# lubaroli/sigsvgd

Hardware: AMD Instinct MI355X
Metric: SVGD iters/sec, sig-kernel N=1024 T=64 d=7 (higher is better)
Workload: dtype f64 static kernel + f32 sweeps and contraction (mixed), f32 I/O

## Files before the change

### sigsvgd_amd/csrc/gram_fast.hip

```cpp
#include <cstdlib>

#include "gram_fast_kernel.h"

namespace sigsvgd {

bool fast_supported(int T, int d, int n) { return n == 0 && T >= 3 && T <= 64 && d <= 16; }
bool fast_wide_supported(int T, int d, int n) { return n == 0 && T >= 3 && T <= 64 && d >= 17 && d <= 32; }

namespace {
inline int grad_nw(int T, int d) { return (d <= 8) ? 8 : 4; }
inline int grad_wg_per_cu(int T, int d) { return (d <= 8 && T <= 32) ? 3 : 1; }
GradGeom fast_geometry(int A, int B, int T, int d, bool sym, int off, int stride, bool fold)
{
    return grad_geometry(A, B, T * d, sym, off, stride, fold, grad_nw(T, d), (long long)device_cu_count() * grad_wg_per_cu(T, d));
}
}

int sym_tile_rows_fast(int T, int d) { return grad_nw(T, d); }

static bool fixed_windows(int T, int want_grad)
{
    if (T != 64 || !want_grad) return false;
    const char *e = getenv("SIGSVGD_SWEEP_WINDOWS");
    return !(e && e[0] == 't');
}

static bool wave_balance(int T, int d, int want_grad, bool sym)
{
    if (!sym || d > 8 || !fast_has_balance<8, true>() || !fixed_windows(T, want_grad)) return false;
    const char *e = getenv("SIGSVGD_WAVE_BALANCE");
    return !(e && e[0] == 'o' && e[1] == 'f');
}

static bool half_offset(int T, int d, int want_grad, bool sym)
{
    if (!sym || d != 7 || !fast_has_half<8, true, true>() || !fixed_windows(T, want_grad)) return false;
    const char *e = getenv("SIGSVGD_HALF_OFFSET");
    return !(e && e[0] == 'o' && e[1] == 'f');
}

WsPlan fast_plan(int A, int B, int T, int d, int want_grad, bool sym, int off, int stride, bool fold, int kind)
{
    WsPlan w;
    const bool rbf = kind == SIGSVGD_STATIC_RBF;
    w.fixed_windows = rbf && d <= 16 && fixed_windows(T, want_grad) ? 1 : 0;
    w.wave_balance = rbf && wave_balance(T, d, want_grad, sym) ? 1 : 0;
    w.half_offset = rbf && half_offset(T, d, want_grad, sym) ? 1 : 0;
    if (d <= 4) w.kflag = w.take(flag_area_bytes(A, B));
    if (want_grad) {
        w.g = fast_geometry(A, B, T, d, sym, off, stride, fold);
        w.rseg = w.take(w.g.rseg_bytes);
        w.cslab = w.take(w.g.cslab_bytes);
    }
    return w;
}

namespace {
int run(const GramProblem &p, const WsPlan &w, bool sym, const TileMap &own, void *out, int out64)
{
    unsigned char *base = nullptr;
    int rc = ws_base(p, w, "fast", base);
    if (rc) return rc;
    FastArgs a{};
    fill_sweep_args(a, p, w, base);
    a.tm = own;
    int tile_rows = 0;
    rc = p.kind != SIGSVGD_STATIC_RBF ? fast_radial_dispatch(p, a, w, out != nullptr, sym, tile_rows)
         : p.d > 16                   ? fast_wide_dispatch(p, a, w, out != nullptr, sym, tile_rows)
                                      : dispatch_variant<0>(p, a, w, out != nullptr, sym, tile_rows);
    if (rc) return rc;
    return finish_launch(p, w, base, sym, a.tm, tile_rows, out, out64);
}
}

int fast_launch(const GramProblem &p)
{
    const bool sym = (p.flags & SIGSVGD_FLAG_Y_IS_X) && p.A == p.B;
    const WsPlan w = fast_plan(p.A, p.B, p.T, p.d, p.gradX_out != nullptr, sym, 0, 1, false, p.kind);
    return run(p, w, sym, make_tilemap(1, 0, 1, false), p.gradX_out, p.dtype == SIGSVGD_F64);
}

int fast_sym_partial(const GramProblem &p, int tile_offset, int tile_stride, bool fold, double *grad_partial)
{
    const WsPlan w = fast_plan(p.A, p.B, p.T, p.d, 1, true, tile_offset, tile_stride, fold, p.kind);
    return run(p, w, true, make_tilemap((p.A + grad_nw(p.T, p.d) - 1) / grad_nw(p.T, p.d), tile_offset, tile_stride, fold),
               grad_partial, 1);
}

}

SIG_EXEC_DEBUG_GETTER(fast)
```

### sigsvgd_amd/csrc/gram_fast_kernel.h

```cpp
#pragma once

#include <type_traits>

#include "sig_common.h"

namespace sigsvgd {

#define SIG_PRIO(n)                                                          \
    if (!GRAD || !SYM || (RING == 32 && NW == 4)) __builtin_amdgcn_s_setprio(n);

template <int BAL>
__device__ __forceinline__ void bal_top(bool first)
{
    if constexpr (BAL != 0) {
        if (first) __builtin_amdgcn_s_setprio(1);
    }
}
template <int BAL, int AT>
__device__ __forceinline__ void bal_switch(bool first)
{
    if constexpr (BAL != 0 && (BAL & 3) == AT) {
        if (first) __builtin_amdgcn_s_setprio(0);
        else __builtin_amdgcn_s_setprio(1);
    }
// ... 253 lines not shown
                     : [cur] "+v"(cur), [upA] "+v"(upA), [upB] "+v"(upB), [V] "+v"(V), [t] "=&v"(t), [y] "=&v"(y),
                       [k0] "+v"(ksl[0]), [k1] "+v"(ksl[1]), [k2] "+v"(ksl[2]), [k3] "+v"(ksl[3]), [k4] "+v"(ksl[4]),
                       [k5] "+v"(ksl[5]), [k6] "+v"(ksl[6]), [k7] "+v"(ksl[7])
                     : [g0] "v"(g[0]), [g1] "v"(g[1]), [g2] "v"(g[2]), [g3] "v"(g[3]), [g4] "v"(g[4]), [g5] "v"(g[5]),
                       [g6] "v"(g[6]), [g7] "v"(g[7]), [r3] "s"(r3), SIG_WIN_OPS(0), SIG_WIN_OPS(1), SIG_WIN_OPS(2),
                       SIG_WIN_OPS(3), SIG_WIN_OPS(4), SIG_WIN_OPS(5), SIG_WIN_OPS(6), SIG_WIN_OPS(7));
    else
        asm volatile(SIG_FWD_STEP_X("upA", "upB", "g0", SIG_FWD_KSL("upB", "k0"), SIG_WIN_FIX("0"))
                     SIG_FWD_STEP_X("upB", "upA", "g1", SIG_FWD_KSL("upA", "k1"), SIG_WIN_FIX("1"))
                     SIG_FWD_STEP_X("upA", "upB", "g2", SIG_FWD_KSL("upB", "k2"), SIG_WIN_FIX("2"))
                     SIG_FWD_STEP_X("upB", "upA", "g3", SIG_FWD_KSL("upA", "k3"), SIG_WIN_FIX("3"))
                     SIG_FWD_STEP_X("upA", "upB", "g4", SIG_FWD_KSL("upB", "k4"), SIG_WIN_FIX("4"))
                     "s_mov_b64 exec, -1\n\t"
                     : [cur] "+v"(cur), [upA] "+v"(upA), [upB] "+v"(upB), [V] "+v"(V), [t] "=&v"(t), [y] "=&v"(y),
                       [k0] "+v"(ksl[0]), [k1] "+v"(ksl[1]), [k2] "+v"(ksl[2]), [k3] "+v"(ksl[3]), [k4] "+v"(ksl[4])
                     : [g0] "v"(g[0]), [g1] "v"(g[1]), [g2] "v"(g[2]), [g3] "v"(g[3]), [g4] "v"(g[4]), [r3] "s"(r3),
                       SIG_WIN_OPS(0), SIG_WIN_OPS(1), SIG_WIN_OPS(2), SIG_WIN_OPS(3), SIG_WIN_OPS(4));
}
template <int PFIX, int SIGMA0, int NS>
__device__ __forceinline__ void sweep_rev_fixed(float &cur, float &dnA, float &dnB, float &V, const float *g, float *ksl, const float r3)
{
    static_assert((NS == 8 || NS == 5) && SIGMA0 % 8 == 0 && SIGMA0 + NS <= 2 * PFIX - 1, "statement shape");
    float t, y;
    SIG_EXEC_MUST_BE_FULL("sweep_rev_fixed");
    if constexpr (NS == 8)
        asm volatile(SIG_REV_STEP_X("dnA", "dnB", "g7", "k7", SIG_WIN_FIX("7")) SIG_REV_STEP_X("dnB", "dnA", "g6", "k6", SIG_WIN_FIX("6"))
                     SIG_REV_STEP_X("dnA", "dnB", "g5", "k5", SIG_WIN_FIX("5")) SIG_REV_STEP_X("dnB", "dnA", "g4", "k4", SIG_WIN_FIX("4"))
                     SIG_REV_STEP_X("dnA", "dnB", "g3", "k3", SIG_WIN_FIX("3")) SIG_REV_STEP_X("dnB", "dnA", "g2", "k2", SIG_WIN_FIX("2"))
                     SIG_REV_STEP_X("dnA", "dnB", "g1", "k1", SIG_WIN_FIX("1")) SIG_REV_STEP_X("dnB", "dnA", "g0", "k0", SIG_WIN_FIX("0"))
                     "s_mov_b64 exec, -1\n\t"
                     : [cur] "+v"(cur), [dnA] "+v"(dnA), [dnB] "+v"(dnB), [V] "+v"(V), [t] "=&v"(t), [y] "=&v"(y),
                       [k0] "+v"(ksl[0]), [k1] "+v"(ksl[1]), [k2] "+v"(ksl[2]), [k3] "+v"(ksl[3]), [k4] "+v"(ksl[4]),
                       [k5] "+v"(ksl[5]), [k6] "+v"(ksl[6]), [k7] "+v"(ksl[7])
                     : [g0] "v"(g[0]), [g1] "v"(g[1]), [g2] "v"(g[2]), [g3] "v"(g[3]), [g4] "v"(g[4]), [g5] "v"(g[5]),
                       [g6] "v"(g[6]), [g7] "v"(g[7]), [r3] "s"(r3), SIG_WIN_OPS(0), SIG_WIN_OPS(1), SIG_WIN_OPS(2),
                       SIG_WIN_OPS(3), SIG_WIN_OPS(4), SIG_WIN_OPS(5), SIG_WIN_OPS(6), SIG_WIN_OPS(7));
    else
        asm volatile(SIG_REV_STEP_X("dnB", "dnA", "g4", "k4", SIG_WIN_FIX("4"))
                     SIG_REV_STEP_X("dnA", "dnB", "g3", "k3", SIG_WIN_FIX("3")) SIG_REV_STEP_X("dnB", "dnA", "g2", "k2", SIG_WIN_FIX("2"))
                     SIG_REV_STEP_X("dnA", "dnB", "g1", "k1", SIG_WIN_FIX("1")) SIG_REV_STEP_X("dnB", "dnA", "g0", "k0", SIG_WIN_FIX("0"))
                     "s_mov_b64 exec, -1\n\t"
                     : [cur] "+v"(cur), [dnA] "+v"(dnA), [dnB] "+v"(dnB), [V] "+v"(V), [t] "=&v"(t), [y] "=&v"(y),
                       [k0] "+v"(ksl[0]), [k1] "+v"(ksl[1]), [k2] "+v"(ksl[2]), [k3] "+v"(ksl[3]), [k4] "+v"(ksl[4])
                     : [g0] "v"(g[0]), [g1] "v"(g[1]), [g2] "v"(g[2]), [g3] "v"(g[3]), [g4] "v"(g[4]), [r3] "s"(r3),
                       SIG_WIN_OPS(0), SIG_WIN_OPS(1), SIG_WIN_OPS(2), SIG_WIN_OPS(3), SIG_WIN_OPS(4));
}
template <int PFIX, int S0, int S1>
__device__ __forceinline__ void sweep_fwd_fixed_round(float &cur, float &upA, float &upB, float &V, const float *Dsl, float *Ksl, const float r3)
{
    if constexpr (S0 < S1) {
        sweep_fwd_fixed<PFIX, S0, (S1 - S0 < 8 ? S1 - S0 : 8)>(cur, upA, upB, V, Dsl + (S0 & 63), Ksl + (S0 & 63), r3);
        sweep_fwd_fixed_round<PFIX, S0 + 8, S1>(cur, upA, upB, V, Dsl, Ksl, r3);
    }
}
template <int PFIX, int S0, int S1>
__device__ __forceinline__ void sweep_rev_fixed_round(float &cur, float &dnA, float &dnB, float &V, const float *Dsl, float *Ksl, const float r3)
{
    if constexpr (S0 < S1) {
        sweep_rev_fixed_round<PFIX, S0 + 8, S1>(cur, dnA, dnB, V, Dsl, Ksl, r3);
        sweep_rev_fixed<PFIX, S0, (S1 - S0 < 8 ? S1 - S0 : 8)>(cur, dnA, dnB, V, Dsl + (S0 & 63), Ksl + (S0 & 63), r3);
    }
}

template <int RING>
__device__ __forceinline__ double resweep_fwd_fp64(const float (&Dsl)[RING], int P, int lrow)
{
    double cur = 1.0, upprev = 1.0;
    asm volatile("" : "+v"(lrow), "+s"(P));
    const bool rowv = lrow < P;
#pragma unroll
    for (int s0 = 0; s0 < 2 * RING - 3; s0 += 8) {
        if (s0 <= 2 * P - 2) {
#pragma unroll
            for (int s = s0; s < s0 + 8 && s < 2 * RING - 3; ++s) {
                const double up = dpp_shr1_one(cur);
                float gf = Dsl[s & (RING - 1)];
                asm volatile("" : "+v"(gf));
                const double g = (double)gf;
                const double t = cur + up;
                const double nw = (t - upprev) + g * __builtin_fma(g, t + upprev, 1.7320508075688772 * t);
                cur = (rowv && (unsigned)(s - lrow) < (unsigned)P) ? nw : cur;
                upprev = up;
            }
        }
    }
    return cur;
}

__device__ __forceinline__ double rsqrt_ge1(double x)
{
    const double y = __builtin_amdgcn_rsq(x);
    const double e = __builtin_fma(-(x * y), y, 1.0);
    return __builtin_fma(y * e, __builtin_fma(e, 0.375, 0.5), y);
}

constexpr int GS_STRIDE = 65;
constexpr int GS_WAVE = 64 * GS_STRIDE;
using f32x2 = __attribute__((ext_vector_type(2))) float;

__device__ __forceinline__ int gs_index(int slot, int lane) { return slot * GS_STRIDE + lane; }

template <int DPAD, int NW, bool GRAD, bool SYM, bool LP, int RING = 64, int PFIX = 0, int BAL = 0, int RADIAL = 0, int HALF = 0>
__global__ __launch_bounds__(NW * 64) __attribute__((amdgpu_waves_per_eu(
    GRAD ? ((RING == 32 && NW == 4 && DPAD <= 8) ? 3 : 1) : ((DPAD <= 8) ? 3 : (DPAD <= 16) ? 2 : 1),
    GRAD ? ((RING == 32 && NW == 4 && DPAD <= 8) ? 3 : (DPAD <= 16) ? 2 : 1) : ((DPAD <= 8) ? 3 : (DPAD <= 16) ? 2 : 1)))) void gram_fast_kernel(FastArgsOf<RADIAL> a)
{
    constexpr int DC = LP ? DPAD - 1 : DPAD;
    constexpr int NT = NW * 64;
    constexpr int RM = RING - 1;
    constexpr int RPW = (RING == 32) ? 2 : 1;
    constexpr int NWR = NW * RPW;
    static_assert(RADIAL == 0 || (PFIX == 0 && BAL == 0), "the radial kinds: general windows, no wave balance");
    static_assert(BAL == 0 || (GRAD && SYM && RING == 64 && NW == 8 && PFIX != 0 && (BAL & 3) != 0 && BAL < 8),
                  "wave balance: the symmetric gradient kernels with fixed windows on 8-wave workgroups (the ones SIG_PRIO leaves alone)");
    static_assert(HALF == 0 || (GRAD && SYM && LP && DPAD == 8 && RING == 64 && NW == 8 && PFIX != 0 && BAL == 0 && RADIAL == 0),
                  "half offset: the symmetric 7-of-8-channel gradient kernel with fixed windows on 8-wave workgroups; a schedule of its own");
    constexpr int YDS = DPAD + 2;
    constexpr int YFS = (DPAD == 4) ? 12 : DPAD + 4;
    constexpr int GSS = HALF ? 64 : GS_STRIDE;
    constexpr int GSW = RING * GSS;
    __shared__ float Gs_all[GRAD ? NW * GSW : 1];
    __shared__ __align__(16) double yd[2 * RING * YDS];
    __shared__ double ynd[HALF ? 1 : 2 * RING];
    constexpr int YFB = 2 * RING * YFS;
    __shared__ double yref[HALF ? 2 * DPAD : DPAD];
    __shared__ __align__(16) float yf[GRAD ? (HALF ? 2 : 1) * YFB : 1];
    __shared__ float ypark[HALF ? (NW / 2) * RING * DC : 1];
    __shared__ float ycarry[HALF ? RING * DC : 1];

    const int tid = threadIdx.x, lane = tid & 63;
    const int wave = __builtin_amdgcn_readfirstlane(tid >> 6);
    const int lrow = lane & RM;
    const bool bal_first = (BAL & 4) ? wave < NW / 2 : wave >= NW / 2;
    const bool half_younger = HALF != 0 && wave >= NW / 2;
    int pb = 0;
    const int T = a.T, d = a.d, P = T - 1, io64 = a.io64;
#ifdef SIGSVGD_PHASE_STAMPS
    unsigned long long ph_[SIG_FAST_PHASES] = {0, 0, 0, 0, 0, 0, 0, 0, 0}, tlast_ = __builtin_amdgcn_s_memtime();
#endif
    int j0 = 0, j1 = 0;
    float *Gs = Gs_all + (GRAD ? wave * GSW : 0);
    const double inv_h = a.inv_h;
    const float m2h = (float)(-2.0 * inv_h * 3.46410161513775459);

    float Ksl[RING];
    double gacc[DPAD];
    double xraw[DPAD];

    constexpr int EPT = (64 * DPAD + NT - 1) / NT;
    constexpr bool RAW_STAGE = GRAD && SYM && RING == 64 && DPAD == 8;
    struct RawElem { unsigned lo, hi; };
    RawElem raw_v[EPT], raw_r[EPT];
    double stage_v[EPT], stage_r[EPT];
    auto load_raw = [&](const void *b, size_t idx) -> RawElem {
        const char *p = static_cast<const char *>(b) + (idx << (io64 ? 3 : 2));
        RawElem r;
        r.lo = *reinterpret_cast<const unsigned *>(p);
        r.hi = 0u;
        if (io64) r.hi = *reinterpret_cast<const unsigned *>(p + 4);
        return r;
    };
    auto raw_value = [&](const RawElem &r) -> double {
        return io64 ? __hiloint2double((int)r.hi, (int)r.lo) : (double)__uint_as_float(r.lo);
    };
    auto stage_load = [&](int j) {
#pragma unroll
        for (int k = 0; k < EPT; ++k) {
            const int e = tid + k * NT;
            const int t = e / DPAD, c = e % DPAD;
            const bool ok = e < RING * DPAD && t < T && c < d && j < a.B;
            if constexpr (RAW_STAGE) {
                raw_v[k] = raw_r[k] = RawElem{0u, 0u};
                if (ok) {
                    raw_v[k] = load_raw(a.Y, ((size_t)j * T + t) * d + c);
                    raw_r[k] = load_raw(a.Y, (size_t)j * T * d + c);
                }
            } else {
                stage_v[k] = ok ? load_any(a.Y, ((size_t)j * T + t) * d + c, io64) : 0.0;
                stage_r[k] = ok ? load_any(a.Y, (size_t)j * T * d + c, io64) : 0.0;
            }
        }
    };
    const double nscale = RADIAL ? inv_h : -inv_h * 1.4426950408889634074;
    auto stage_store = [&](int buf) {
#pragma unroll
        for (int k = 0; k < EPT; ++k) {
            const int e = tid + k * NT;
            if (e < RING * DPAD) {
                const int t = e / DPAD, c = e % DPAD;
                if constexpr (RAW_STAGE) {
                    stage_v[k] = raw_value(raw_v[k]);
                    stage_r[k] = raw_value(raw_r[k]);
                }
                const double v = stage_v[k] - stage_r[k];
                if (!(LP && c == DPAD - 1)) {
                    yd[t * YDS + c] = v;
                    yd[(t + RING) * YDS + c] = v;
                }
                if (GRAD) {
                    float *yfb = yf + (HALF ? buf * YFB : 0);
                    yfb[t * YFS + c] = (float)v;
                    yfb[(t + RING) * YFS + c] = (float)v;
                }
                if (t == 0) yref[(HALF ? buf * DPAD : 0) + c] = stage_r[k];
                double s = v * v * nscale;
#pragma unroll
                for (int off = 1; off < DPAD; off <<= 1) s += __shfl_xor(s, off, 64);
                if (c == 0) {
                    if constexpr (!HALF) {
                        ynd[t] = s;
                        ynd[t + RING] = s;
                    }
                    if (LP) {
                        yd[t * YDS + DPAD - 1] = s;
                        yd[(t + RING) * YDS + DPAD - 1] = s;
                    }
                }
            }
        }
    };

    const long long it0 = a.nitems * blockIdx.x / gridDim.x, it1 = a.nitems * (blockIdx.x + 1) / gridDim.x;
    int remaining = (int)(it1 - it0);
    long long item = it0;
    int kq = 0, cstart = 0;
    {
        long long rem = it0;
        for (;; ++kq) {
            const int cn = a.B - (SYM ? a.tm.tile_of(kq) * NWR : 0);
            if (rem < cn) break;
            rem -= cn;
        }
        cstart = (int)rem;
    }
    bool staged = false;
    while (remaining > 0) {
    const int itile = a.tm.tile_of(kq);
    const int cfirst = SYM ? itile * NWR : 0;
    const int ncol = min(a.B - cfirst - cstart, remaining);
    const int jnext_tile = SYM ? a.tm.tile_of(kq + 1) * NWR : 0;
    const bool more_tiles = remaining > ncol;
    const int i0 = itile * NWR + wave * RPW;
    const int i = (RING == 32) ? i0 + (lane >> 5) : i0;
    const bool row_ok = i < a.A;
#pragma unroll
    for (int c = 0; c < DPAD; ++c) {
        gacc[c] = 0.0;
        xraw[c] = (row_ok && lrow < T && c < d) ? load_any(a.X, ((size_t)i * T + lrow) * d + c, io64) : 0.0;
    }
    if constexpr (RAW_STAGE) {
#pragma unroll
        for (int c = 0; c < DPAD; ++c) asm volatile("" : "+v"(xraw[c]));
    }
    j0 = cfirst + cstart;
    j1 = j0 + ncol;
    if (!staged) {
        staged = true;
        stage_load(j0);
        stage_store(pb);
        __syncthreads();
    }

    for (int j = j0; j < j1; ++j) {
        const bool pair_ok = i0 < a.A && (!SYM || j >= i0);
        const bool mine = row_ok && (!SYM || j >= i);
        const bool last = j + 1 == j1;
        const bool more = !last || more_tiles;
        if (more) stage_load(last ? jnext_tile : j + 1);

        float Dsl[RING];
        const double *yrefp = yref + (HALF ? pb * DPAD : 0);
        auto pair_sync = [&]() __attribute__((always_inline)) {
            SIG_STAMP(5)
#ifndef SIG_EXPERIMENT_NO_PAIR_BARRIER
            __syncthreads();
#endif
            SIG_STAMP(6)
            if constexpr (HALF != 0) {
                const float inv_d = 1.0f / (float)d;
                const bool pend = j > j0;
                float *dstp = a.cslab + (size_t)(item - 1) * (T * d);
                for (int e = tid; e < T * d; e += NT) {
                    const int n = (int)(((float)e + 0.5f) * inv_d), c = e - n * d;
                    if (pend) {
                        float s = ycarry[e];
#pragma unroll
                        for (int w = 0; w < NW / 2; ++w) s += ypark[w * RING * DC + e];
                        dstp[e] = s;
                    }
                    float s = 0.f;
#pragma unroll
                    for (int w = 0; w < NW / 2; ++w) s += Gs_all[w * GSW + n * DPAD + c];
                    ycarry[e] = s;
                }
            } else if (GRAD && SYM) {
                const float inv_d = 1.0f / (float)d;
                float *dst = a.cslab + (size_t)item * (T * d);
                for (int e = tid; e < T * d; e += NT) {
                    const int n = (int)(((float)e + 0.5f) * inv_d), c = e - n * d;
                    float s = 0.f;
#pragma unroll
                    for (int w = 0; w < NW; ++w) {
                        s += Gs_all[w * GSW + n * DPAD + c];
                        if (RING == 32) s += Gs_all[w * GSW + (RING + n) * DPAD + c];
                    }
                    dst[e] = s;
                }
            }
            ++item;
            if (more) stage_store(HALF ? pb ^ 1 : 0);
            SIG_STAMP(7)
#ifndef SIG_EXPERIMENT_NO_PAIR_BARRIER
            __syncthreads();
#endif
            SIG_STAMP(8)
        };
        auto younger_sync = [&]() __attribute__((always_inline)) {
            if constexpr (RAW_STAGE) {
#pragma unroll
                for (int k = 0; k < EPT; ++k)
                    asm volatile("" : "+v"(raw_v[k].lo), "+v"(raw_v[k].hi), "+v"(raw_r[k].lo), "+v"(raw_r[k].hi));
            }
            pair_sync();
        };

        SIG_STAMP(0)
        SIG_PRIO(3)
        if (pair_ok) {
            bal_top<BAL>(bal_first);
            double xs[DPAD];
            double xn = 0.0;
#pragma unroll
            for (int c = 0; c < DPAD; ++c) {
                const double xc = (lrow < T && c < d) ? xraw[c] - yrefp[c] : 0.0;
                xn = __builtin_fma(xc, xc, xn);
                xs[c] = xc * (-2.0 * nscale);
            }
// ... 243 lines not shown
                    const unsigned long long *mk = (RING == 64 ? SWEEP_MASK.m[P] : SWEEP_MASK32.m[P]) + rnd * 64;
#pragma unroll
                    for (int k0 = 56; k0 >= 0; k0 -= 8) sweep_rev8(cur, downA, downB, V, &Dsl[k0 & RM], &Ksl[k0 & RM], mk + k0, r3);
                }

                if constexpr (DPAD == 4) {
                    if (a.kflag) {
                        float cs = 0.f;
#pragma unroll
                        for (int k = 0; k < RING; ++k) cs = __builtin_fmaf(fabsf(Ksl[k]), fabsf(Dsl[k]), cs);
                        const float wsum = wave_sum_dpp<RING == 64>(cs);
                        float c1 = __int_as_float(__builtin_amdgcn_readlane(__float_as_int(wsum), 63));
                        if (RING == 32) {
                            const float c10 = __int_as_float(__builtin_amdgcn_readlane(__float_as_int(wsum), 31));
                            c1 = (lane >> 5) ? c1 : c10;
                        }
                        const bool ill = kf_keep == kf_keep && c1 * 3.46410161513775459f > 150.f * fmaxf(fabsf(kf_keep), 0.1f);
                        if (lrow == P - 1 && mine)
                            a.kflag[(size_t)i * a.B + j] = (((RING == 32 && (lane >> 5)) ? x1_keep : x0_keep) || ill) ? 1 : 0;
                    }
                }
                SIG_STAMP(3)
                SIG_PRIO(0)
                float gnx = 0.f, Svn = Ksl[RM];
                f32x2 ynx[DPAD / 2];
#pragma unroll
                for (int c = 0; c < DPAD / 2; ++c) ynx[c] = f32x2{0.f, 0.f};
                if constexpr (DPAD > 16) {
#pragma clang loop unroll(full)
                for (int it = 0; it < RING + 2; ++it) {
                    const float Sv = Svn, gcu = gnx;
                    f32x2 ycu[DPAD / 2];
#pragma unroll
                    for (int c = 0; c < DPAD / 2; ++c) ycu[c] = ynx[c];
                    if (it + 1 < RING + 2) {
                        Svn = Ksl[(RING - 2 - it) & RM];
                        if (it + 1 >= 2) {
                            const int k2n = (RING - it) & RM;
                            gnx = Gs_all[gsoff + k2n * GSS];
                            const f32x2 *yr = reinterpret_cast<const f32x2 *>(yf + (yfrow + k2n) * YFS);
#pragma unroll
                            for (int c = 0; c < DPAD / 2; ++c) ynx[c] = yr[c];
                        }
                    }
                    grad_part(Sv, it >= 2, gcu, ycu);
                    __builtin_amdgcn_sched_barrier(0);
                }
                } else {
#pragma unroll
                for (int it = 0; it < RING + 2; ++it) {
                    const float Sv = Svn, gcu = gnx;
                    f32x2 ycu[DPAD / 2];
#pragma unroll
                    for (int c = 0; c < DPAD / 2; ++c) ycu[c] = ynx[c];
                    if (it + 1 < RING + 2) {
                        Svn = Ksl[(RING - 2 - it) & RM];
                        if (it + 1 >= 2) {
                            const int k2n = (RING - it) & RM;
                            gnx = Gs_all[gsoff + k2n * GSS];
                            const f32x2 *yr = reinterpret_cast<const f32x2 *>(yf + (yfrow + k2n) * YFS);
#pragma unroll
                            for (int c = 0; c < DPAD / 2; ++c) ynx[c] = yr[c];
                        }
                    }
                    grad_part(Sv, it >= 2, gcu, ycu);
                    __builtin_amdgcn_sched_barrier(0);
                }
                }

                SIG_STAMP(4)
#pragma unroll
                for (int c = 0; c < DPAD; ++c) {
                    gacc[c] += (double)(w_ij * m2h * acc[c / 2][c % 2]);
                }

                if (SYM) {
                    const int ncol = (RING - lrow) & RM;
                    const float wpark = (ncol <= P) ? ((RING == 32) ? -m2h : -(wcol * m2h)) : 0.f;
                    if (HALF != 0 && half_younger) {
                        float *pk = ypark + ((wave - NW / 2) * RING + ncol) * DC;
#pragma unroll
                        for (int c = 0; c < DC; ++c) pk[c] = wpark * tacc[c];
                    } else {
                    float *pk = Gs + ((RING == 32 ? (lane >> 5) * RING : 0) + ncol) * DPAD;
#pragma unroll
                    for (int c = 0; c < DPAD; ++c) pk[c] = wpark * tacc[c];
                    }
                }
            }
        } else if (GRAD && SYM) {
            if (HALF != 0 && half_younger) {
                younger_sync();
#pragma unroll
                for (int c = 0; c < DC; ++c) ypark[((wave - NW / 2) * RING + lane) * DC + c] = 0.f;
            } else {
#pragma unroll
            for (int c = 0; c < DPAD; ++c) Gs[lane * DPAD + c] = 0.f;
            }
        }
        if constexpr (RAW_STAGE) {
#pragma unroll
            for (int k = 0; k < EPT; ++k)
                asm volatile("" : "+v"(raw_v[k].lo), "+v"(raw_v[k].hi), "+v"(raw_r[k].lo), "+v"(raw_r[k].hi));
        }
        bal_end<BAL>(bal_first);
        if constexpr (HALF != 0) __builtin_amdgcn_s_setprio(0);
        if (!half_younger) pair_sync();
        if constexpr (HALF != 0) pb ^= 1;
    }
    if constexpr (HALF != 0) {
        __syncthreads();
        float *dstp = a.cslab + (size_t)(item - 1) * (T * d);
        for (int e = tid; e < T * d; e += NT) {
            float s = ycarry[e];
#pragma unroll
            for (int w = 0; w < NW / 2; ++w) s += ypark[w * RING * DC + e];
            dstp[e] = s;
        }
    }

    if (GRAD && row_ok && lrow < T) {
        const int rslot = wave * RPW + (RING == 32 ? (lane >> 5) : 0);
        double *dst = a.rseg + (((size_t)(kq + (int)blockIdx.x)) * NWR + rslot) * (size_t)(T * d) + lrow * d;
#pragma unroll
        for (int c = 0; c < DPAD; ++c)
            if (c < d) dst[c] = gacc[c];
    }
    remaining -= ncol;
    ++kq;
    cstart = 0;
    }
#ifdef SIGSVGD_PHASE_STAMPS
    SIG_STAMP(0)
    if (lane == 0 && a.stamps)
        for (int k = 0; k < SIG_FAST_PHASES; ++k) atomicAdd(&a.stamps[(wave >= NW / 2 ? SIG_FAST_PHASES : 0) + k], ph_[k]);
#endif
}

#ifndef SIG_EXPERIMENT_BALANCE
#define SIG_EXPERIMENT_BALANCE 6
#endif
constexpr int FAST_BAL = SIG_EXPERIMENT_BALANCE;
template <int DPAD, bool SYM>
constexpr bool fast_has_balance() { return FAST_BAL != 0 && SYM && DPAD <= 8; }

template <int DPAD, bool SYM, bool LP>
constexpr bool fast_has_half() { return SYM && LP && DPAD == 8; }

int fast_radial_dispatch(const GramProblem &p, FastArgs &a, const WsPlan &w, bool grad, bool sym, int &tile_rows);
int fast_wide_dispatch(const GramProblem &p, FastArgs &a, const WsPlan &w, bool grad, bool sym, int &tile_rows);

namespace {
template <int DPAD, int NW, bool SYM, bool LP, int RING, int RADIAL>
void launch_grad(bool fix, bool bal, bool half, dim3 grid, dim3 block, hipStream_t stream, const FastArgsOf<RADIAL> &a)
{
    if constexpr (RADIAL == 0 && RING == 64 && DPAD <= 16 && NW == (DPAD <= 8 ? 8 : 4)) {
        if constexpr (fast_has_half<DPAD, SYM, LP>()) {
            if (fix && half) {
                hipLaunchKernelGGL((gram_fast_kernel<DPAD, NW, true, SYM, LP, RING, 63, 0, 0, 1>), grid, block, 0, stream, a);
                return;
            }
        }
        if constexpr (fast_has_balance<DPAD, SYM>()) {
            if (fix && bal) {
                hipLaunchKernelGGL((gram_fast_kernel<DPAD, NW, true, SYM, LP, RING, 63, FAST_BAL>), grid, block, 0, stream, a);
                return;
            }
        }
        if (fix) {
            hipLaunchKernelGGL((gram_fast_kernel<DPAD, NW, true, SYM, LP, RING, 63>), grid, block, 0, stream, a);
            return;
        }
    }
    hipLaunchKernelGGL((gram_fast_kernel<DPAD, NW, true, SYM, LP, RING, 0, 0, RADIAL>), grid, block, 0, stream, a);
}

template <int RADIAL, int DPAD, int NW, int RING = 64>
int launch_variant(const GramProblem &p, FastArgs &a, const WsPlan &w, bool grad, bool sym, int &tile_rows)
{
    constexpr int NWR = NW * (RING == 32 ? 2 : 1);
    tile_rows = NWR;
    const TileMap tm = make_tilemap((p.A + NWR - 1) / NWR, a.tm.off, a.tm.stride, a.tm.fold != 0);
    if (tm.owned <= 0) return SIGSVGD_OK;
    const long long total = tm.start(tm.owned, p.B, NWR, sym ? 1 : 0);
    if (total <= 0) return SIGSVGD_OK;
    const int ncu = device_cu_count();
    a.tm = tm;
    a.nitems = total;
#ifdef SIGSVGD_PHASE_STAMPS
    a.stamps = phase_stamps_begin(p.stream);
#endif
    const long long resident = (long long)ncu * (grad ? ((RING == 32 && NW == 4 && DPAD <= 8) ? 3 : 1) : (NW == 4 ? ((DPAD <= 8) ? 3 : (DPAD <= 16) ? 2 : 1) : 1));
    dim3 grid((unsigned)(total < resident ? total : resident), 1);
    dim3 block(NW * 64);
    if (grad) {
        const GradGeom &g = w.g;
        if (g.NW != NWR || g.grid != (int)grid.x || g.nitems != total) {
            set_error("fast: launch geometry mismatch (rows per tile %d/%d grid %d/%u items %lld/%lld)", g.NW, NWR, g.grid, grid.x,
                      g.nitems, total);
            return SIGSVGD_E_BADARG;
        }
    }
    constexpr bool HAS_LP = DPAD <= 8 || DPAD == 32;
    const bool lp = HAS_LP && grad && p.d == DPAD - 1;
    FastArgsOf<RADIAL> ka{};
    static_cast<FastArgs &>(ka) = a;
    if constexpr (RADIAL != 0) ka.kind = p.kind;
    const bool fix = grad && w.fixed_windows && p.T == 64;
    const bool bal = fix && w.wave_balance;
    const bool half = fix && w.half_offset;
    if (!grad && sym)
        hipLaunchKernelGGL((gram_fast_kernel<DPAD, NW, false, true, false, RING, 0, 0, RADIAL>), grid, block, 0, p.stream, ka);
    else if (!grad)
        hipLaunchKernelGGL((gram_fast_kernel<DPAD, NW, false, false, false, RING, 0, 0, RADIAL>), grid, block, 0, p.stream, ka);
    else if (sym && lp)
        launch_grad<DPAD, NW, true, HAS_LP, RING, RADIAL>(fix, bal, half, grid, block, p.stream, ka);
    else if (sym)
        launch_grad<DPAD, NW, true, false, RING, RADIAL>(fix, bal, half, grid, block, p.stream, ka);
    else if (lp)
        launch_grad<DPAD, NW, false, HAS_LP, RING, RADIAL>(fix, bal, half, grid, block, p.stream, ka);
    else
        launch_grad<DPAD, NW, false, false, RING, RADIAL>(fix, bal, half, grid, block, p.stream, ka);
    hipError_t e = hipGetLastError();
    if (e != hipSuccess) return hip_fail(e, "launch gram_fast_kernel");
#ifdef SIGSVGD_PHASE_STAMPS
    static const char *const nm[] = {"loop top", "phase 0+1 static kernel", "phase 2 forward sweep", "phase 3 reverse sweep",
                                      "phase 4 gradient pass", "pair epilogue", "barrier after the pair",
                                      "block sum + stage store", "second barrier"};
    static_assert(sizeof(nm) / sizeof(nm[0]) == SIG_FAST_PHASES, "one name per stamp slot");
    phase_stamps_report_halves(p.stream, a.stamps, nm, "[phase stamps] A=%d T=%d d=%d grad=%d sym=%d: ", p.A, p.T, p.d, (int)grad, (int)sym);
#endif
    return SIGSVGD_OK;
}

template <int RADIAL>
int dispatch_variant(const GramProblem &p, FastArgs &a, const WsPlan &w, bool grad, bool sym, int &tile_rows)
{
    if (!grad && p.d <= 4)
        return p.T <= 32 ? launch_variant<RADIAL, 4, 4, 32>(p, a, w, false, sym, tile_rows) : launch_variant<RADIAL, 4, 4>(p, a, w, false, sym, tile_rows);
    if (!grad && p.d <= 8)
        return p.T <= 32 ? launch_variant<RADIAL, 8, 4, 32>(p, a, w, false, sym, tile_rows) : launch_variant<RADIAL, 8, 4>(p, a, w, false, sym, tile_rows);
    if (p.d <= 4)
        return p.T <= 32 ? launch_variant<RADIAL, 4, 4, 32>(p, a, w, grad, sym, tile_rows) : launch_variant<RADIAL, 4, 8>(p, a, w, grad, sym, tile_rows);
    if (p.d <= 8)
        return p.T <= 32 ? launch_variant<RADIAL, 8, 4, 32>(p, a, w, grad, sym, tile_rows) : launch_variant<RADIAL, 8, 8>(p, a, w, grad, sym, tile_rows);
    return launch_variant<RADIAL, 16, 4>(p, a, w, grad, sym, tile_rows);
}
}
}
```

### sigsvgd_amd/csrc/sig_common.h

```cpp
#pragma once
#include <hip/hip_runtime.h>
#include <stdint.h>

#include <atomic>
#ifdef SIGSVGD_PHASE_STAMPS
#include <cstdarg>
#include <cstdio>
#endif

#include "../../include/sigsvgd_hip.h"

namespace sigsvgd {

constexpr int kWave = 64;

void set_error(const char *fmt, ...);
int hip_fail(hipError_t e, const char *what);

__device__ __forceinline__ double exp64(double a0)
{
    double a = fmin(fmax(a0, -1000.0), 700.0);
    const double kf = __builtin_rint(a * 1.4426950408889634074);
    double r = __builtin_fma(kf, -6.93147180369123816490e-01, a);
    r = __builtin_fma(kf, -1.90821492927058770002e-10, r);
// ... 116 lines not shown
}

#ifdef SIGSVGD_PHASE_STAMPS
#define SIG_STAMP(i)                                                         \
    {                                                                        \
        const unsigned long long now_ = __builtin_amdgcn_s_memtime();        \
        ph_[i] += now_ - tlast_;                                             \
        tlast_ = now_;                                                       \
    }
constexpr int kMaxPhases = 32;
inline unsigned long long *phase_stamps_begin(hipStream_t stream)
{
    static unsigned long long *buf = nullptr;
    if (!buf) (void)hipMalloc(&buf, kMaxPhases * sizeof(unsigned long long));
    (void)hipMemsetAsync(buf, 0, kMaxPhases * sizeof(unsigned long long), stream);
    return buf;
}
template <int N>
void phase_stamps_report(hipStream_t stream, const unsigned long long *buf, const char *const (&names)[N], const char *fmt, ...)
{
    static_assert(N <= kMaxPhases, "more phases than the buffer holds");
    unsigned long long h[kMaxPhases];
    (void)hipStreamSynchronize(stream);
    (void)hipMemcpy(h, buf, sizeof(h), hipMemcpyDeviceToHost);
    double tot = 0;
    for (int k = 0; k < kMaxPhases; ++k) tot += (double)h[k];
    va_list ap;
    va_start(ap, fmt);
    vfprintf(stderr, fmt, ap);
    va_end(ap);
    for (int k = 0; k < N; ++k) fprintf(stderr, "%s %.1f%% | ", names[k], 100.0 * (double)h[k] / tot);
    fprintf(stderr, "total %.3e wave-cycles\n", tot);
}
template <int N>
void phase_stamps_report_halves(hipStream_t stream, const unsigned long long *buf, const char *const (&names)[N], const char *fmt, ...)
{
    static_assert(2 * N <= kMaxPhases, "more phases than the buffer holds");
    unsigned long long h[kMaxPhases];
    (void)hipStreamSynchronize(stream);
    (void)hipMemcpy(h, buf, sizeof(h), hipMemcpyDeviceToHost);
    double tot[2] = {0, 0};
    for (int k = 0; k < N; ++k) {
        tot[0] += (double)h[k];
        tot[1] += (double)h[N + k];
    }
    char head[256];
    va_list ap;
    va_start(ap, fmt);
    vsnprintf(head, sizeof(head), fmt, ap);
    va_end(ap);
    fprintf(stderr, "%s", head);
    for (int k = 0; k < N; ++k) fprintf(stderr, "%s %.1f%% | ", names[k], 100.0 * (double)(h[k] + h[N + k]) / (tot[0] + tot[1]));
    fprintf(stderr, "total %.3e wave-cycles\n", tot[0] + tot[1]);
    fprintf(stderr, "%solder | younger half: ", head);
    for (int k = 0; k < N; ++k)
        fprintf(stderr, "%s %.1f%% | %.1f%% ; ", names[k], 100.0 * (double)h[k] / tot[0], 100.0 * (double)h[N + k] / tot[1]);
    fprintf(stderr, "total %.3e | %.3e wave-cycles\n", tot[0], tot[1]);
}
#else
#define SIG_STAMP(i)
#endif

#ifdef SIGSVGD_CHECK_EXEC
static __device__ unsigned g_exec_violations;
#define SIG_EXEC_MUST_BE_FULL(what)                                                        \
    do {                                                                                   \
        if (__builtin_amdgcn_read_exec() != ~0ull) g_exec_violations = 1u;                 \
    } while (0)
#define SIG_EXEC_DEBUG_GETTER(unit)                                                        \
    extern "C" unsigned sigsvgd_debug_exec_violations_##unit(void)                         \
    {                                                                                      \
        unsigned v = 0xffffffffu;                                                          \
        (void)hipDeviceSynchronize();                                                      \
        (void)hipMemcpyFromSymbol(&v, HIP_SYMBOL(sigsvgd::g_exec_violations), sizeof(v));  \
        return v;                                                                          \
    }
#else
#define SIG_EXEC_MUST_BE_FULL(what)
#define SIG_EXEC_DEBUG_GETTER(unit)
#endif

struct GramProblem {
    const void *X, *Y;
    int A, B, T, d, dtype;
    double inv_h;
    int n;
    int kind;
    unsigned flags;
    const void *grad_out;
    void *K_out;
    void *gradX_out;
    void *ws;
    size_t ws_bytes;
    hipStream_t stream;
};

struct LongProblem {
    const void *X, *Y;
    int A, B, TX, TY, d, dtype;
    double inv_h;
    int n;
    int kind;
    unsigned flags;
    const void *grad_out;
    void *K_out;
    void *gradX_out, *gradY_out;
    void *ws;
    size_t ws_bytes;
    hipStream_t stream;
};

struct TileMap {
    int off, stride, ntile, owned, m0, fold;
    __host__ __device__ int tile_of(int kq) const
    {
        return kq < m0 ? off + kq * stride : ntile - 1 - (off + (kq - m0) * stride);
    }
    __host__ __device__ int kq_of_tile(int ti) const
    {
        if (ti >= off && (ti - off) % stride == 0 && (ti - off) / stride < m0) return (ti - off) / stride;
        const int p = ntile - 1 - ti;
        if (p >= off && (p - off) % stride == 0 && (p - off) / stride < owned - m0) return m0 + (p - off) / stride;
        return -1;
    }
    __host__ __device__ long long start(int kq, int B, int NW, int sym) const
    {
        if (!sym) return (long long)kq * B;
        const long long k1 = kq < m0 ? kq : m0, k2 = kq - k1;
        long long s = k1 * B - (long long)NW * ((long long)stride * k1 * (k1 - 1) / 2 + (long long)off * k1);
        s += k2 * ((long long)B - (long long)(ntile - 1 - off) * NW) + (long long)NW * stride * k2 * (k2 - 1) / 2;
        return s;
    }
};
TileMap make_tilemap(int ntile, int off, int stride, bool fold);

struct GradGeom {
    int NW, grid;
    TileMap tm;
    long long nitems;
    size_t rseg_bytes, cslab_bytes;
};
int device_cu_count();
GradGeom grad_geometry(int A, int B, int TD, bool sym, int off, int stride, bool fold, int NW, long long resident);
int grad_reduce_launch(const GradGeom &g, const double *rseg, const float *cslab, void *out, int out64, int A, int B, int TD,
                       bool sym, hipStream_t stream);

struct WsArea {
    size_t off = 0, bytes = 0;
};
struct WsPlan {
    GradGeom g{};
    WsArea kflag;
    WsArea rseg, cslab;
    WsArea crec, rowg, dcache;
    WsArea wsk;
    WsArea counter, partials, colslab;
    int fixed_windows = 0;
    int wave_balance = 0;
    int half_offset = 0;
    size_t end = 0;
    WsArea take(size_t bytes)
    {
        const WsArea a{end, bytes};
        end += bytes;
        return a;
    }
    size_t total() const { return end + 256; }
};
inline size_t flag_area_bytes(int A, int B) { return ((size_t)A * B + 255) & ~(size_t)255; }
template <typename T>
inline T *ws_at(unsigned char *base, const WsArea &a)
{
    return a.bytes ? reinterpret_cast<T *>(base + a.off) : nullptr;
}
int ws_base(const GramProblem &p, const WsPlan &w, const char *family, unsigned char *&base);
int finish_launch(const GramProblem &p, const WsPlan &w, unsigned char *base, bool sym, const TileMap &tm, int tile_rows,
                  void *out, int out64);

template <typename Args>
void fill_sweep_args(Args &a, const GramProblem &p, const WsPlan &w, unsigned char *base)
{
    a.X = p.X; a.Y = p.Y; a.go = p.grad_out; a.K = p.K_out;
    a.kflag = ws_at<unsigned char>(base, w.kflag); a.rseg = ws_at<double>(base, w.rseg); a.cslab = ws_at<float>(base, w.cslab);
    a.io64 = p.dtype == SIGSVGD_F64; a.A = p.A; a.B = p.B; a.T = p.T; a.d = p.d;
    a.symw = (p.flags & SIGSVGD_FLAG_SYM) ? 1 : 0; a.inv_h = p.inv_h;
}

template <auto KERNEL>
hipError_t raise_lds_limit()
{
    static std::atomic<unsigned long long> raised{0};
    int dev = 0;
    (void)hipGetDevice(&dev);
    if (dev < 0 || dev >= 64 || !((raised.load(std::memory_order_acquire) >> dev) & 1ull)) {
        hipError_t e = hipFuncSetAttribute(reinterpret_cast<const void *>(KERNEL), hipFuncAttributeMaxDynamicSharedMemorySize,
                                           160 * 1024);
        if (e != hipSuccess) return e;
        if (dev >= 0 && dev < 64) raised.fetch_or(1ull << dev, std::memory_order_release);
    }
    return hipSuccess;
}


int generic_plan(int A, int B, int T, int d, int n, int want_grad, bool sym, bool precise, bool any_size, WsPlan &w);
int generic_launch(const GramProblem &p, bool precise, bool any_size);
int generic_repair_launch(const GramProblem &p, const unsigned char *flags, bool sym, const TileMap &tm, int tile_rows);

bool fast_supported(int T, int d, int n);
bool fast_wide_supported(int T, int d, int n);
WsPlan fast_plan(int A, int B, int T, int d, int want_grad, bool sym, int off = 0, int stride = 1, bool fold = false,
                 int kind = SIGSVGD_STATIC_RBF);
int fast_launch(const GramProblem &p);
int fast_sym_partial(const GramProblem &p, int tile_offset, int tile_stride, bool fold, double *grad_partial);
int sym_tile_rows_fast(int T, int d);

bool quad_supported(int T, int d, int n);
WsPlan quad_plan(int A, int B, int T, int d, int want_grad, bool sym, int off = 0, int stride = 1, bool fold = false);
int quad_launch(const GramProblem &p);
int quad_sym_partial(const GramProblem &p, int tile_offset, int tile_stride, bool fold, double *grad_partial);

bool dyad_supported(int T, int d, int n);
WsPlan dyad_plan(int A, int B, int T, int d, int want_grad, bool sym);
int dyad_launch(const GramProblem &p);

bool band_supported(int T, int d, int n);
int band_wg_per_cu(int T, int d, int n, bool serial);
WsPlan band_plan(int A, int B, int T, int d, int n, int want_grad, bool sym, bool serial);
int band_launch(const GramProblem &p, bool serial);

}
```

Baseline: 222.3.

## Precompute per-column path images in a prepass kernel for staged loads

Adds a small prepass kernel that converts each column path into a contiguous f64 image holding the increments relative to the first point, a per-timestep scaled squared norm in the padding lane, and the reference point. The main gram kernel gets a new HALF==2 variant that loads this image with one aligned 8-byte load per thread instead of scattered f32 loads and subtractions. The aim is to cut staging work and uncoalesced global reads inside the hot sweep loop. The cost is an extra kernel launch and workspace per call. The padding lane now carries the norm in the f64 tile but is zeroed in the f32 tile, so any consumer of that lane must expect this layout.

```diff
diff --git a/sigsvgd_amd/csrc/gram_fast.hip b/sigsvgd_amd/csrc/gram_fast.hip
--- a/sigsvgd_amd/csrc/gram_fast.hip
+++ b/sigsvgd_amd/csrc/gram_fast.hip
@@ -39,6 +39,44 @@
     return !(e && e[0] == 'o' && e[1] == 'f');
 }
 
+static bool column_images()
+{
+    const char *e = getenv("SIGSVGD_COLUMN_IMAGES");
+    return !(e && e[0] == 'o' && e[1] == 'f');
+}
+
+constexpr int COLIMG_DOUBLES = 64 * 8 + 8;
+inline size_t colimg_bytes(int B) { return ((size_t)B * COLIMG_DOUBLES * sizeof(double) + 255) & ~(size_t)255; }
+
+__device__ __forceinline__ double column_norm(double v, double nscale)
+{
+#pragma clang fp contract(off)
+    const double vv = v * v;
+    const double s = vv * nscale;
+    double r = __builtin_fma(nscale, vv, __shfl_xor(s, 1, 64));
+    r = r + __shfl_xor(r, 2, 64);
+    r = r + __shfl_xor(r, 4, 64);
+    return r;
+}
+
+__global__ __launch_bounds__(512) void fast_column_image_kernel(const void *Y, double *img, int io64, double inv_h)
+{
+    constexpr int T = 64, d = 7, DPAD = 8;
+    const int j = blockIdx.x, e = threadIdx.x, t = e / DPAD, c = e % DPAD;
+    const double nscale = -inv_h * 1.4426950408889634074;
+    double sv = 0.0, sr = 0.0;
+    if (c < d) {
+        sv = load_any(Y, ((size_t)j * T + t) * d + c, io64);
+        sr = load_any(Y, (size_t)j * T * d + c, io64);
+    }
+    const double v = sv - sr;
+    const double s = column_norm(v, nscale);
+    double *o = img + (size_t)j * COLIMG_DOUBLES;
+    if (c < d) o[e] = v;
+    if (c == 0) o[e + DPAD - 1] = s;
+    if (t == 0) o[T * DPAD + c] = sr;
+}
+
 WsPlan fast_plan(int A, int B, int T, int d, int want_grad, bool sym, int off, int stride, bool fold, int kind)
 {
     WsPlan w;
@@ -52,6 +90,8 @@
         w.rseg = w.take(w.g.rseg_bytes);
         w.cslab = w.take(w.g.cslab_bytes);
     }
+    w.column_images = w.half_offset && column_images() ? 1 : 0;
+    if (half_offset(T, d, want_grad, sym) && column_images()) w.colimg = w.take(colimg_bytes(B));
     return w;
 }
 
@@ -64,6 +104,13 @@
     FastArgs a{};
     fill_sweep_args(a, p, w, base);
     a.tm = own;
+    if (w.column_images) {
+        double *img = ws_at<double>(base, w.colimg);
+        hipLaunchKernelGGL(fast_column_image_kernel, dim3((unsigned)p.B), dim3(512), 0, p.stream, p.Y, img, a.io64, p.inv_h);
+        hipError_t e = hipGetLastError();
+        if (e != hipSuccess) return hip_fail(e, "launch fast_column_image_kernel");
+        a.Y = img;
+    }
     int tile_rows = 0;
     rc = p.kind != SIGSVGD_STATIC_RBF ? fast_radial_dispatch(p, a, w, out != nullptr, sym, tile_rows)
          : p.d > 16                   ? fast_wide_dispatch(p, a, w, out != nullptr, sym, tile_rows)
diff --git a/sigsvgd_amd/csrc/gram_fast_kernel.h b/sigsvgd_amd/csrc/gram_fast_kernel.h
--- a/sigsvgd_amd/csrc/gram_fast_kernel.h
+++ b/sigsvgd_amd/csrc/gram_fast_kernel.h
@@ -429,6 +429,13 @@
     struct RawElem { unsigned lo, hi; };
     RawElem raw_v[EPT], raw_r[EPT];
     double stage_v[EPT], stage_r[EPT];
+    constexpr bool IMG = HALF == 2;
+    constexpr int IMG_DOUBLES = 64 * 8 + 8;
+#ifdef SIG_EXPERIMENT_STAGE_COPY
+    constexpr bool STAGE_COPY = HALF == 1;
+#else
+    constexpr bool STAGE_COPY = false;
+#endif
     auto load_raw = [&](const void *b, size_t idx) -> RawElem {
         const char *p = static_cast<const char *>(b) + (idx << (io64 ? 3 : 2));
         RawElem r;
@@ -441,6 +448,30 @@
         return io64 ? __hiloint2double((int)r.hi, (int)r.lo) : (double)__uint_as_float(r.lo);
     };
     auto stage_load = [&](int j) {
+        if constexpr (IMG) {
+            static_assert(EPT == 1 && NT == 64 * DPAD, "column images: thread e holds element e");
+            raw_v[0] = raw_r[0] = RawElem{0u, 0u};
+            if (j < a.B) {
+                const uint2 *img = reinterpret_cast<const uint2 *>(static_cast<const double *>(a.Y) + (size_t)j * IMG_DOUBLES);
+                const uint2 w = img[tid];
+                raw_v[0] = RawElem{w.x, w.y};
+                if (tid < DPAD) {
+                    const uint2 r = img[64 * DPAD + tid];
+                    raw_r[0] = RawElem{r.x, r.y};
+                }
+            }
+            return;
+        }
+        if constexpr (STAGE_COPY) {
+            static_assert(EPT == 1, "stage copy: one element per thread");
+            raw_v[0] = raw_r[0] = RawElem{0u, 0u};
+            if (j < a.B) {
+                const uint2 w = *reinterpret_cast<const uint2 *>(static_cast<const char *>(a.Y) + (size_t)j * (64 * 7 * 4) +
+                                                                 (size_t)(((tid & 127) + ((tid >> 7) & 1) * 96) * 8));
+                raw_v[0] = RawElem{w.x, w.y};
+            }
+            return;
+        }
 #pragma unroll
         for (int k = 0; k < EPT; ++k) {
             const int e = tid + k * NT;
@@ -460,6 +491,29 @@
     };
     const double nscale = RADIAL ? inv_h : -inv_h * 1.4426950408889634074;
     auto stage_store = [&](int buf) {
+        if constexpr (IMG) {
+            const int t = tid / DPAD, c = tid % DPAD;
+            const double v = __hiloint2double((int)raw_v[0].hi, (int)raw_v[0].lo);
+            yd[t * YDS + c] = v;
+            yd[(t + RING) * YDS + c] = v;
+            const float vf = (c == DPAD - 1) ? 0.f : (float)v;
+            float *yfb = yf + buf * YFB;
+            yfb[t * YFS + c] = vf;
+            yfb[(t + RING) * YFS + c] = vf;
+            if (t == 0) yref[buf * DPAD + c] = __hiloint2double((int)raw_r[0].hi, (int)raw_r[0].lo);
+            return;
+        }
+        if constexpr (STAGE_COPY) {
+            const int t = tid / DPAD, c = tid % DPAD;
+            const double v = __hiloint2double((int)((raw_v[0].hi & 0x800FFFFFu) | 0x3F500000u), (int)raw_v[0].lo);
+            yd[t * YDS + c] = v;
+            yd[(t + RING) * YDS + c] = v;
+            float *yfb = yf + buf * YFB;
+            yfb[t * YFS + c] = __uint_as_float(raw_v[0].lo);
+            yfb[(t + RING) * YFS + c] = __uint_as_float(raw_v[0].lo);
+            if (t == 0) yref[buf * DPAD + c] = v;
+            return;
+        }
 #pragma unroll
         for (int k = 0; k < EPT; ++k) {
             const int e = tid + k * NT;
@@ -1009,10 +1063,14 @@
 
 namespace {
 template <int DPAD, int NW, bool SYM, bool LP, int RING, int RADIAL>
-void launch_grad(bool fix, bool bal, bool half, dim3 grid, dim3 block, hipStream_t stream, const FastArgsOf<RADIAL> &a)
+void launch_grad(bool fix, bool bal, bool half, bool img, dim3 grid, dim3 block, hipStream_t stream, const FastArgsOf<RADIAL> &a)
 {
     if constexpr (RADIAL == 0 && RING == 64 && DPAD <= 16 && NW == (DPAD <= 8 ? 8 : 4)) {
         if constexpr (fast_has_half<DPAD, SYM, LP>()) {
+            if (fix && half && img) {
+                hipLaunchKernelGGL((gram_fast_kernel<DPAD, NW, true, SYM, LP, RING, 63, 0, 0, 2>), grid, block, 0, stream, a);
+                return;
+            }
             if (fix && half) {
                 hipLaunchKernelGGL((gram_fast_kernel<DPAD, NW, true, SYM, LP, RING, 63, 0, 0, 1>), grid, block, 0, stream, a);
                 return;
@@ -1066,18 +1124,19 @@
     const bool fix = grad && w.fixed_windows && p.T == 64;
     const bool bal = fix && w.wave_balance;
     const bool half = fix && w.half_offset;
+    const bool img = half && w.column_images;
     if (!grad && sym)
         hipLaunchKernelGGL((gram_fast_kernel<DPAD, NW, false, true, false, RING, 0, 0, RADIAL>), grid, block, 0, p.stream, ka);
     else if (!grad)
         hipLaunchKernelGGL((gram_fast_kernel<DPAD, NW, false, false, false, RING, 0, 0, RADIAL>), grid, block, 0, p.stream, ka);
     else if (sym && lp)
-        launch_grad<DPAD, NW, true, HAS_LP, RING, RADIAL>(fix, bal, half, grid, block, p.stream, ka);
+        launch_grad<DPAD, NW, true, HAS_LP, RING, RADIAL>(fix, bal, half, img, grid, block, p.stream, ka);
     else if (sym)
-        launch_grad<DPAD, NW, true, false, RING, RADIAL>(fix, bal, half, grid, block, p.stream, ka);
+        launch_grad<DPAD, NW, true, false, RING, RADIAL>(fix, bal, half, img, grid, block, p.stream, ka);
     else if (lp)
-        launch_grad<DPAD, NW, false, HAS_LP, RING, RADIAL>(fix, bal, half, grid, block, p.stream, ka);
+        launch_grad<DPAD, NW, false, HAS_LP, RING, RADIAL>(fix, bal, half, img, grid, block, p.stream, ka);
     else
-        launch_grad<DPAD, NW, false, false, RING, RADIAL>(fix, bal, half, grid, block, p.stream, ka);
+        launch_grad<DPAD, NW, false, false, RING, RADIAL>(fix, bal, half, img, grid, block, p.stream, ka);
     hipError_t e = hipGetLastError();
     if (e != hipSuccess) return hip_fail(e, "launch gram_fast_kernel");
 #ifdef SIGSVGD_PHASE_STAMPS
diff --git a/sigsvgd_amd/csrc/sig_common.h b/sigsvgd_amd/csrc/sig_common.h
--- a/sigsvgd_amd/csrc/sig_common.h
+++ b/sigsvgd_amd/csrc/sig_common.h
@@ -292,12 +292,14 @@
     GradGeom g{};
     WsArea kflag;
     WsArea rseg, cslab;
+    WsArea colimg;
     WsArea crec, rowg, dcache;
     WsArea wsk;
     WsArea counter, partials, colslab;
     int fixed_windows = 0;
     int wave_balance = 0;
     int half_offset = 0;
+    int column_images = 0;
     size_t end = 0;
     WsArea take(size_t bytes)
     {
```

Result: faster. 226.2 (median of 6 runs) (+1.8%).
